# nmndeep/Robust-Segmentation

Measured on AMD Instinct MI355X. Metric: SEA attack-iterations/sec (UperNet-CNX-T, 512x512), higher is better.
Workload: dtype f32 (frozen-weight GEMMs on the 16-bit matrix cores by operand splitting: fp16x2 (22 significant bits per operand, 3 MFMA products) forward, fp16x2 (22 significant bits per operand, 3 MFMA products) input gradient; fp32 storage and accumulate)

## Files before the change

include/sea_hip.h:

```cpp
#ifndef SEA_HIP_H
#define SEA_HIP_H

#include <stddef.h>
#include <stdint.h>

#ifdef __cplusplus
extern "C" {
#endif

#define SEA_MODE_MASK_CE 0
#define SEA_MODE_MASK_CE_BAL 1
#define SEA_MODE_JS 2
#define SEA_MODE_CE 3

#define SEA_DTYPE_F32 0
#define SEA_DTYPE_BF16 1
#define SEA_DTYPE_F16 2

#define SEA_LAYOUT_NCHW 0
#define SEA_LAYOUT_NHWC 1

int sea_abi_version(void);
const char* sea_build_info(void);
#define SEA_CONFIG_XCD_ORDER 0
// ... 41 lines not shown
                     int64_t* tgt_cnt, void* stream);
int sea_confusion(const void* pred, int pred_bytes, const void* y, int y_bytes, int64_t n, int C,
                  int64_t* hist, void* stream);

int sea_apgd_track(const float* loss_sum, const float* track_sum, const int32_t* n_correct,
                   const int32_t* n_ignored, int B, int64_t HW, int iter, int n_iter, int check_k,
                   int early_stop, int init, int32_t* acc_cnt, float* acc, float* loss_best,
                   float* loss_best_last, float* reduced_last, float* step, float* loss_steps,
                   uint8_t* flags, int32_t* done, const void* loss_workspace, void* stream);
int sea_apgd_linf_step_graph(const float* x, float* x_adv, float* x_old, const float* grad, const float* step_b,
                             const float* eps_dev, const int32_t* iter_dev, int B, int64_t n_per_img, void* stream);
int sea_apgd_track_graph(const float* loss_sum, const float* track_sum, const int32_t* n_correct,
                         const int32_t* n_ignored, int B, int64_t HW, int32_t* iter_dev, const int32_t* check_table,
                         const int32_t* n_iter_dev, int early_stop, int32_t* acc_cnt, float* acc, float* loss_best,
                         float* loss_best_last, float* reduced_last, float* step, float* loss_steps, uint8_t* flags,
                         int32_t* done, const void* loss_workspace, void* stream);
int sea_select_copy(const uint8_t* flags, float* x_adv, float* grad, float* x_best,
                    float* grad_best, float* x_best_adv, const void* pred, void* pred_best,
                    int pred_bytes, int B, int64_t n_per_img, int64_t HW, void* stream);

int sea_count_ignored(const void* y, int y_bytes, int B, int64_t HW, int32_t* n_ignored,
                      void* stream);

int sea_worst_miou_greedy(const float* ints, const float* unions, int A, int N, int C,
                          uint32_t* mt_state, int n_rounds, double* miou, int32_t* selected,
                          int32_t* rounds_run);

int sea_dwconv7x7(const float* x, const float* w, const float* bias, float* y, int B, int C, int H,
                  int W, int flip, void* stream);
int sea_dwconv7x7_nhwc(const float* x, const float* wt, const float* bias, float* y, int B, int C,
                       int H, int W, int flip, unsigned ab, void* stream);
int sea_dwconv7x7_nhwc_add(const float* x, const float* wt, const float* bias, const float* addend, float* y, int B,
                           int C, int H, int W, int flip, unsigned ab, void* stream);

int sea_upsample_bilinear_fwd(const float* x, float* y, int64_t planes, int h, int w, int H, int W,
                              void* stream);
int sea_upsample_bilinear_bwd(const float* gy, float* gx, int64_t planes, int h, int w, int H, int W,
                              void* stream);
int sea_upsample_bilinear_nhwc_fwd(const float* x, const float* residual, float* y, int B, int C, int h,
                                   int w, int H, int W, int64_t y_pixel_stride, void* stream);
int sea_upsample_bilinear_nhwc_bwd(const float* gy, float* gx, int B, int C, int h, int w, int H, int W,
                                   int64_t gy_pixel_stride, void* stream);

int64_t sea_wino_tiles(int B, int H, int W, int m);
int sea_wino_input_transform(const float* x, int64_t x_pixel_stride, const float* gate, const float* scale,
                             float* V, int64_t v_tile_stride, int B, int C, int H, int W, int m, int vec4, void* stream);
int sea_wino_filter_transform(const float* w, float* U, int Cout, int Cin, int m, int flip, void* stream);
int sea_wino_input_transform_amax(const float* x, int64_t x_pixel_stride, const float* gate, const float* scale, float* V,
                                  int64_t v_tile_stride, int B, int C, int H, int W, int m, int vec4, uint32_t* amax_out,
                                  void* stream);
int sea_wino_output_transform(const float* M, const float* addend, const float* scale, const float* bias,
                              int relu, float* y, int B, int C, int H, int W, int m, int vec4, void* stream);

int sea_layernorm_fwd(const float* x, const float* w, const float* b, float* y, float* mean, float* rstd,
                      int64_t rows, int C, float eps, void* stream);
int sea_layernorm_bwd(const float* g, const float* x, const float* w, const float* mean, const float* rstd,
                      float* dx, int64_t rows, int C, void* stream);

int64_t sea_dwconv7x7_nhwc_wgrad_workspace(int B, int C, int H);
int sea_dwconv7x7_nhwc_wgrad(const float* x, const float* gy, float* gw, float* gb, float* ws, int B, int C, int H, int W,
                             void* stream);

int sea_adaptive_avg_pool_nhwc_fwd(const float* x, float* out, int B, int C, int H, int W, int oh, int ow, void* stream);
int sea_adaptive_avg_pool_nhwc_bwd(const float* g, float* dx, int B, int C, int H, int W, int oh, int ow, void* stream);

int sea_stem_conv1_ln_gelu(const float* x, const float* w, const float* bias, const float* gamma, const float* beta,
// ... 131 lines not shown
```

robust-segmentation_amd/csrc/dwconv_kernels.hip:

```cpp
#include "sea_common.h"

namespace sea {

constexpr int DW_T = 32;
constexpr int DW_K = 7, DW_P = 3;
constexpr int DW_IN = DW_T + DW_K - 1;
constexpr int DW_LD = 40;

template <bool FLIP, bool BIAS>
__global__ __launch_bounds__(256) void dwconv7x7_kernel(const float* __restrict__ x, const float* __restrict__ w,
                                                        const float* __restrict__ bias, float* __restrict__ y,
                                                        int C, int H, int W, int tiles_x) {
  __shared__ __attribute__((aligned(16))) float tile[DW_IN * DW_LD];
  const int plane = blockIdx.y;
  const int c = plane % C;
  const int ty0 = (blockIdx.x / tiles_x) * DW_T, tx0 = (blockIdx.x % tiles_x) * DW_T;
  const float* xp = x + (int64_t)plane * H * W;
  for (int i = threadIdx.x; i < DW_IN * DW_IN; i += 256) {
    const int r = i / DW_IN, q = i - r * DW_IN;
    const int gy = ty0 + r - DW_P, gx = tx0 + q - DW_P;
    float v = 0.f;
    if (gy >= 0 && gy < H && gx >= 0 && gx < W) v = xp[(int64_t)gy * W + gx];
    tile[r * DW_LD + q] = v;
  }
// ... 146 lines not shown
    float4 w[DW_K];
    load_input_row(oy0 - DW_P + r, in);
    if (r < DW_K) {
      load_filter_row(r, w);
      accumulate(in, w, acc0);
    }
    __builtin_amdgcn_sched_barrier(0);
    if (r >= 1) {
      load_filter_row(r - 1, w);
      accumulate(in, w, acc1);
    }
    __builtin_amdgcn_sched_barrier(0);
  }
  const int64_t ro = ((int64_t)b * H + oy0) * W * CG + cg;
  float4* yr = y + ro;
#pragma unroll
  for (int j = 0; j < DWN_STRIP; ++j)
    if (ox0 + j < W) {
      if (ADD) acc0[j] = add4(acc0[j], addend[ro + (int64_t)(ox0 + j) * CG]);
      yr[(int64_t)(ox0 + j) * CG] = acc0[j];
    }
  if (oy0 + 1 < H) {
#pragma unroll
    for (int j = 0; j < DWN_STRIP; ++j)
      if (ox0 + j < W) {
        if (ADD) acc1[j] = add4(acc1[j], addend[ro + ((int64_t)W + ox0 + j) * CG]);
        yr[((int64_t)W + ox0 + j) * CG] = acc1[j];
      }
  }
}

typedef float dw_f4 __attribute__((ext_vector_type(4)));

template <int CG, int ROWS, bool FLIP, bool BIAS, bool ADD, bool WLDS>
__global__ __launch_bounds__(256, 2) void dwconv7x7_nhwc_pipe_kernel(const float4* __restrict__ x, const float4* __restrict__ wt,
                                                                     const float4* __restrict__ bias,
                                                                     const float4* __restrict__ addend, float4* __restrict__ y,
                                                                     int H, int W, int gx, int HP, int units, int per_xcd) {
  constexpr int SPB = 256 / CG, NIN = DWN_STRIP + DW_K - 1;
  constexpr uint32_t OOB = 0x40000000u;
  extern __shared__ __attribute__((aligned(16))) char dw_smem[];
  const int cg = threadIdx.x % CG, ps = threadIdx.x / CG;
  const int u = per_xcd ? (int)(blockIdx.x % 8) * per_xcd + (int)(blockIdx.x / 8) : (int)blockIdx.x;
  if (u >= units) return;
  if constexpr (WLDS) {
    for (int i = threadIdx.x; i < DW_K * DW_K * CG; i += 256) {
      const int tap = i / CG, c = i - tap * CG;
      *(float4*)(dw_smem + i * 16) = wt[(FLIP ? (DW_K * DW_K - 1 - tap) : tap) * CG + c];
    }
    __syncthreads();
  }
  if (ps >= SPB) return;
  const int bx = u % gx, op = (u / gx) % HP, b = u / (gx * HP);
  const int oy0 = op * ROWS;
  const int ox0 = (bx * SPB + ps) * DWN_STRIP;
  if (ox0 >= W) return;
  const int row_bytes = W * CG * 16;
  const char* const img = (const char*)(x + (int64_t)b * H * W * CG);
  const uint32_t vbase = (uint32_t)((ox0 * CG + cg) * 16);
  const float4* const wb = wt + cg;

  dw_f4 in[2][NIN], w[2][DW_K];
  auto load_input_row = [&](int iy, dw_f4 (&dst)[NIN]) __attribute__((always_inline)) {
    const bool ok = iy >= 0 && iy < H;
    const __amdgpu_buffer_rsrc_t rs =
        __builtin_amdgcn_make_buffer_rsrc((void*)(img + (int64_t)(ok ? iy : 0) * row_bytes), 0, ok ? row_bytes : 0, 0x00020000);
#pragma unroll
    for (int j = 0; j < NIN; ++j) {
      uint32_t off;
      if (j < DW_P)
        off = ox0 > 0 ? vbase - (uint32_t)((DW_P - j) * CG * 16) : OOB;
      else
        off = vbase + (uint32_t)((j - DW_P) * CG * 16);
      dst[j] = __builtin_bit_cast(dw_f4, __builtin_amdgcn_raw_buffer_load_b128(rs, (int)off, 0, 0));
    }
  };
  auto load_filter_row = [&](int ky, dw_f4 (&dst)[DW_K]) __attribute__((always_inline)) {
#pragma unroll
    for (int kx = 0; kx < DW_K; ++kx) {
      const int tap = ky * DW_K + kx;
      if constexpr (WLDS)
        dst[kx] = *(const dw_f4*)(dw_smem + (tap * CG + cg) * 16);
      else
        dst[kx] = *(const dw_f4*)(wb + (FLIP ? (DW_K * DW_K - 1 - tap) : tap) * CG);
// ... 28 lines not shown
      if (r >= 1) accumulate(in[cur], w[cur ^ 1], acc1);
      __builtin_amdgcn_sched_barrier(0);
      if (r + 1 < DW_K) load_filter_row(r + 1, w[cur ^ 1]);
      __builtin_amdgcn_sched_barrier(0);
      if (r < DW_K) accumulate(in[cur], w[cur], acc0);
      __builtin_amdgcn_sched_barrier(0);
    }
  } else {
#pragma unroll
    for (int r = 0; r < DW_K; ++r) {
      const int cur = r & 1;
      if (r + 1 < DW_K) {
        load_input_row(oy0 - DW_P + r + 1, in[cur ^ 1]);
        load_filter_row(r + 1, w[cur ^ 1]);
      }
      __builtin_amdgcn_sched_barrier(0);
      accumulate(in[cur], w[cur], acc0);
      __builtin_amdgcn_sched_barrier(0);
    }
  }
  const int64_t ro = ((int64_t)b * H + oy0) * W * CG + cg;
  dw_f4* const yr = (dw_f4*)(y + ro);
#pragma unroll
  for (int j = 0; j < DWN_STRIP; ++j) {
    if (ADD) acc0[j] += *(const dw_f4*)(addend + ro + (int64_t)(ox0 + j) * CG);
    yr[(int64_t)(ox0 + j) * CG] = acc0[j];
  }
  if constexpr (ROWS == 2) {
#pragma unroll
    for (int j = 0; j < DWN_STRIP; ++j) {
      if (ADD) acc1[j] += *(const dw_f4*)(addend + ro + ((int64_t)W + ox0 + j) * CG);
      yr[((int64_t)W + ox0 + j) * CG] = acc1[j];
    }
  }
}

}

using namespace sea;

template <int CG, int ROWS, bool FLIP, bool BIAS, bool ADD>
static void dw_pipe_launch(dim3 grid, hipStream_t s, const float4* x4, const float4* w4, const float4* b4, const float4* a4,
                           float4* y4, int H, int W, int gx, int HP, int units, int per_xcd, bool wlds) {
  if constexpr (CG <= 96) {
    if (wlds) {
      constexpr int lds = DW_K * DW_K * CG * 16;
      auto k = dwconv7x7_nhwc_pipe_kernel<CG, ROWS, FLIP, BIAS, ADD, true>;
      if constexpr (lds > 65536) {
        static bool attr_set_dev[64] = {};
        int dev = 0;
        (void)hipGetDevice(&dev);
        if (!attr_set_dev[dev & 63]) {
          (void)hipFuncSetAttribute((const void*)k, hipFuncAttributeMaxDynamicSharedMemorySize, lds);
          attr_set_dev[dev & 63] = true;
        }
      }
      hipLaunchKernelGGL(k, grid, dim3(256), (size_t)lds, s, x4, w4, b4, a4, y4, H, W, gx, HP, units, per_xcd);
      return;
    }
  }
  hipLaunchKernelGGL((dwconv7x7_nhwc_pipe_kernel<CG, ROWS, FLIP, BIAS, ADD, false>), grid, dim3(256), 0, s, x4, w4, b4, a4, y4, H, W,
                     gx, HP, units, per_xcd);
}

extern "C" int sea_dwconv7x7_nhwc_add(const float* x, const float* wt, const float* bias, const float* addend, float* y,
                                      int B, int C, int H, int W, int flip, unsigned ab, void* stream) {
  SEA_CHECK_ARG(ab < 128 && !(ab & 1));
  SEA_CHECK_ARG(x && wt && y && B > 0 && B <= 65535 && C > 0 && (C % 4) == 0 && C <= 1024 && H > 0 && H <= 65535 && W > 0);
  SEA_CHECK_ARG(((((uintptr_t)x) | ((uintptr_t)wt) | ((uintptr_t)y) | ((uintptr_t)bias) | ((uintptr_t)addend)) & 15) == 0);
  SEA_CHECK_ARG(!(addend && bias));
  const int CG = C / 4;
  const int spb = 256 / CG;
  const int strips = (W + DWN_STRIP - 1) / DWN_STRIP;
  const int gx = (strips + spb - 1) / spb;
  hipStream_t s = (hipStream_t)stream;
  const float4 *x4 = (const float4*)x, *w4 = (const float4*)wt, *b4 = (const float4*)bias, *a4 = (const float4*)addend;
  float4* y4 = (float4*)y;
  const int CG0 = C / 4;
  const bool pipe_ok = !(ab & 16) && (CG0 == 24 || CG0 == 48 || CG0 == 96 || CG0 == 192) && (int64_t)B * H * W * C * 4 < (1ll << 31) &&
                       (W % DWN_STRIP) == 0;
  const bool two_rows = !(ab & 4) && H >= 2 && ((ab & 8) || (int64_t)H * W >= (pipe_ok && (H % 2) == 0 ? 1024 : 4096));
  const int HP = two_rows ? (H + 1) / 2 : H;
  const int64_t units64 = (int64_t)gx * HP * B;
  SEA_CHECK_ARG(units64 < (1ll << 30));
  const int units = (int)units64;
  const int per_xcd = (ab & 2) ? 0 : (units + 7) / 8;
  dim3 grid(per_xcd ? per_xcd * 8 : units), block(256);
#define SEA_DW_LAUNCH(F, BI, AD)                                                                                        \
  do {                                                                                                                  \
    if (two_rows)                                                                                                       \
      hipLaunchKernelGGL((dwconv7x7_nhwc_2row_kernel<F, BI, AD>), grid, block, 0, s, x4, w4, b4, a4, y4, CG, H, W, spb,  \
                         gx, HP, units, per_xcd);                                                                       \
    else                                                                                                                \
      hipLaunchKernelGGL((dwconv7x7_nhwc_kernel<F, BI, AD>), grid, block, 0, s, x4, w4, b4, a4, y4, CG, H, W, spb, gx,   \
                         units, per_xcd);                                                                               \
  } while (0)
  const bool piped = pipe_ok && (!two_rows || (H % 2) == 0);
#define SEA_DW_PIPE(CGV, F, BI, AD)                                                              \
  do {                                                                                           \
    if (two_rows)                                                                                \
      dw_pipe_launch<CGV, 2, F, BI, AD>(grid, s, x4, w4, b4, a4, y4, H, W, gx, HP, units, per_xcd, wlds); \
    else                                                                                         \
      dw_pipe_launch<CGV, 1, F, BI, AD>(grid, s, x4, w4, b4, a4, y4, H, W, gx, HP, units, per_xcd, wlds); \
  } while (0)
  const bool wlds = !(ab & 32) && (!two_rows || (ab & 64));
#define SEA_DW_PIPE_CG(F, BI, AD)                       \
  do {                                                  \
    if (CG == 24) SEA_DW_PIPE(24, F, BI, AD);           \
    else if (CG == 48) SEA_DW_PIPE(48, F, BI, AD);      \
    else if (CG == 96) SEA_DW_PIPE(96, F, BI, AD);      \
    else SEA_DW_PIPE(192, F, BI, AD);                   \
  } while (0)
  if (piped) {
    if (flip) {
      if (addend) SEA_DW_PIPE_CG(true, false, true); else SEA_DW_PIPE_CG(true, false, false);
    } else if (bias) {
      SEA_DW_PIPE_CG(false, true, false);
    } else if (addend) {
      SEA_DW_PIPE_CG(false, false, true);
    } else {
      SEA_DW_PIPE_CG(false, false, false);
    }
    SEA_RETURN_LAST();
  }
#undef SEA_DW_PIPE_CG
#undef SEA_DW_PIPE
  if (flip) {
    if (addend)
      SEA_DW_LAUNCH(true, false, true);
    else
      SEA_DW_LAUNCH(true, false, false);
  } else if (bias) {
    SEA_DW_LAUNCH(false, true, false);
  } else if (addend) {
    SEA_DW_LAUNCH(false, false, true);
  } else {
    SEA_DW_LAUNCH(false, false, false);
  }
#undef SEA_DW_LAUNCH
  SEA_RETURN_LAST();
}

namespace sea {
__global__ __launch_bounds__(448) void dwconv7x7_nhwc_wgrad_partial_kernel(const float4* __restrict__ x,
                                                                           const float4* __restrict__ gy,
// ... 91 lines not shown
  return R < 1 ? 1 : (R > 8 ? 8 : R);
}
static inline int dw_wgrad_chunks(int tiles) { return tiles >= 64 ? 32 : 1; }

extern "C" int64_t sea_dwconv7x7_nhwc_wgrad_workspace(int B, int C, int H) {
  if (B <= 0 || C <= 0 || H <= 0) return 0;
  const int R = dw_wgrad_rows(B, C, H);
  const int64_t tiles = (int64_t)B * ((H + R - 1) / R);
  return (tiles + 32) * 50 * C;
}

extern "C" int sea_dwconv7x7_nhwc_wgrad(const float* x, const float* gy, float* gw, float* gb, float* ws, int B, int C,
                                        int H, int W, void* stream) {
  SEA_CHECK_ARG(x && gy && gw && ws && B > 0 && C > 0 && (C % 4) == 0 && H > 0 && W > 0);
  SEA_CHECK_ARG(((((uintptr_t)x) | ((uintptr_t)gy) | ((uintptr_t)ws)) & 15) == 0);
  const int R = dw_wgrad_rows(B, C, H), tpi = (H + R - 1) / R;
  SEA_CHECK_ARG((int64_t)B * tpi < (1ll << 31));
  const int tiles = B * tpi, chunks = dw_wgrad_chunks(tiles), per = (tiles + chunks - 1) / chunks;
  hipStream_t st = (hipStream_t)stream;
  hipLaunchKernelGGL(dwconv7x7_nhwc_wgrad_partial_kernel, dim3(tiles, (C / 4 + 63) / 64), dim3(448), 0, st, (const float4*)x,
                     (const float4*)gy, (float4*)ws, C / 4, H, W, R, tpi);
  const dim3 g1((50 * C + 255) / 256, chunks), g2((50 * C + 255) / 256, 1);
  if (chunks > 1) {
    float* ws2 = ws + (int64_t)tiles * 50 * C;
    hipLaunchKernelGGL(dwconv7x7_nhwc_wgrad_reduce_kernel, g1, dim3(256), 0, st, (const float*)ws, ws2, (float*)nullptr,
                       (float*)nullptr, C, tiles, per);
    hipLaunchKernelGGL(dwconv7x7_nhwc_wgrad_reduce_kernel, g2, dim3(256), 0, st, (const float*)ws2, (float*)nullptr, gw, gb, C,
                       chunks, chunks);
  } else {
    hipLaunchKernelGGL(dwconv7x7_nhwc_wgrad_reduce_kernel, g2, dim3(256), 0, st, (const float*)ws, (float*)nullptr, gw, gb, C, tiles,
                       tiles);
  }
  SEA_RETURN_LAST();
}

extern "C" int sea_dwconv7x7_nhwc(const float* x, const float* wt, const float* bias, float* y, int B, int C, int H,
                                  int W, int flip, unsigned ab, void* stream) {
  return sea_dwconv7x7_nhwc_add(x, wt, bias, nullptr, y, B, C, H, W, flip, ab, stream);
}

extern "C" int sea_dwconv7x7(const float* x, const float* w, const float* bias, float* y, int B, int C, int H, int W,
                             int flip, void* stream) {
  SEA_CHECK_ARG(x && w && y && B > 0 && C > 0 && H > 0 && W > 0);
  const int64_t planes = (int64_t)B * C;
  SEA_CHECK_ARG(planes <= 65535 * 16);
  const int tiles_x = (W + DW_T - 1) / DW_T, tiles_y = (H + DW_T - 1) / DW_T;
  SEA_CHECK_ARG(planes <= 2147483647 / 1 && (int64_t)tiles_x * tiles_y <= 2147483647);
  hipStream_t s = (hipStream_t)stream;
  const int64_t chunk = 65535;
  for (int64_t p0 = 0; p0 < planes; p0 += chunk) {
    const int np = (int)((planes - p0) < chunk ? (planes - p0) : chunk);
    SEA_CHECK_ARG(p0 % C == 0 || planes <= chunk);
    dim3 grid(tiles_x * tiles_y, np);
    const float* xs = x + p0 * H * W;
    float* ys = y + p0 * H * W;
    if (flip)
      hipLaunchKernelGGL((dwconv7x7_kernel<true, false>), grid, dim3(256), 0, s, xs, w, (const float*)nullptr, ys, C, H, W, tiles_x);
    else if (bias)
      hipLaunchKernelGGL((dwconv7x7_kernel<false, true>), grid, dim3(256), 0, s, xs, w, bias, ys, C, H, W, tiles_x);
    else
      hipLaunchKernelGGL((dwconv7x7_kernel<false, false>), grid, dim3(256), 0, s, xs, w, (const float*)nullptr, ys, C, H, W, tiles_x);
  }
  SEA_RETURN_LAST();
}
```

robust-segmentation_amd/semseg/_native.py:

```python
from __future__ import annotations

import ctypes as C
import os
from typing import Optional

import torch

_PKG = os.path.dirname(os.path.dirname(os.path.abspath(__file__)))
LIB_PATH = os.environ.get("SEA_HIP_LIB", os.path.join(_PKG, "lib", "libsea_hip.so"))

MODE_BY_NAME = {"mask-ce-avg": 0, "mask-ce-bal": 1, "js-avg": 2, "ce": 3, "ce-avg": 3}
DTYPE_CODE = {torch.float32: 0, torch.bfloat16: 1, torch.float16: 2}
LAYOUT_NCHW, LAYOUT_NHWC = 0, 1

_lib = None

_vp, _i, _i64, _f, _sz, _u = C.c_void_p, C.c_int, C.c_int64, C.c_float, C.c_size_t, C.c_uint
_SIGS = {
    "sea_abi_version": (C.c_int, []),
    "sea_build_info": (C.c_char_p, []),
    "sea_fastdiv_magic": (_i, [C.c_uint32, C.POINTER(C.c_uint32), C.POINTER(C.c_uint32)]),
    "sea_apgd_linf_step": (_i, [_vp, _vp, _vp, _vp, _vp, _f, _f, _vp, _i, _i64, _vp]),
    "sea_apgd_l2_workspace_bytes": (_i64, [_i]),
    "sea_apgd_l2_step": (_i, [_vp, _vp, _vp, _vp, _vp, _f, _f, _vp, _vp, _i, _i64, _vp]),
    "sea_linf_random_start": (_i, [_vp, _vp, _f, _vp, _i64, _vp]),
    "sea_linf_project": (_i, [_vp, _vp, _f, _vp, _i64, _vp]),
    "sea_pgd_linf_step": (_i, [_vp, _vp, _vp, _f, _f, _vp, _vp, _i, _i64, _vp]),
    "sea_loss_workspace_bytes": (_sz, [_i, _i64]),
    "sea_loss_fwd_bwd": (_i, [_vp, _i, _i, _vp, _i, _vp, _i, _i, _i, _i, _i64, _f, _vp, _vp, _i, _vp, _vp, _sz,
                              _vp, _vp, _vp, _vp]),
    "sea_loss_fwd_bwd_tuned": (_i, [_vp, _i, _i, _vp, _i, _vp, _i, _i, _i, _i, _i64, _f, _vp, _vp, _i, _vp, _vp,
                                    _sz, _vp, _vp, _vp, _vp, _i]),
    "sea_loss_upsampled_workspace_bytes": (_sz, [_i, _i, _i, _i, _i, _i, _i]),
    "sea_loss_fwd_bwd_upsampled": (_i, [_vp, _vp, _i, _vp, _i, _i, _i, _i, _i, _i, _i, _i, _f, _vp, _vp, _i, _vp, _sz, _vp,
                                        _vp, _vp, _i, _vp]),
    "sea_class_counts": (_i, [_vp, _i, _vp, _i, _i, _i, _i64, _i, _i, _vp, _vp, _vp, _vp]),
    "sea_confusion": (_i, [_vp, _i, _vp, _i, _i64, _i, _vp, _vp]),
    "sea_apgd_track": (_i, [_vp, _vp, _vp, _vp, _i, _i64, _i, _i, _i, _i, _i, _vp, _vp, _vp, _vp, _vp, _vp, _vp,
                            _vp, _vp, _vp, _vp]),
    "sea_apgd_linf_step_graph": (_i, [_vp, _vp, _vp, _vp, _vp, _vp, _vp, _i, _i64, _vp]),
    "sea_apgd_track_graph": (_i, [_vp, _vp, _vp, _vp, _i, _i64, _vp, _vp, _vp, _i, _vp, _vp, _vp, _vp, _vp, _vp, _vp, _vp,
                                  _vp, _vp, _vp]),
    "sea_select_copy": (_i, [_vp, _vp, _vp, _vp, _vp, _vp, _vp, _vp, _i, _i, _i64, _i64, _vp]),
    "sea_count_ignored": (_i, [_vp, _i, _i, _i64, _vp, _vp]),
    "sea_worst_miou_greedy": (_i, [_vp, _vp, _i, _i, _i, _vp, _i, _vp, _vp, _vp]),
    "sea_dwconv7x7": (_i, [_vp, _vp, _vp, _vp, _i, _i, _i, _i, _i, _vp]),
    "sea_dwconv7x7_nhwc": (_i, [_vp, _vp, _vp, _vp, _i, _i, _i, _i, _i, _u, _vp]),
    "sea_dwconv7x7_nhwc_add": (_i, [_vp, _vp, _vp, _vp, _vp, _i, _i, _i, _i, _i, _u, _vp]),
    "sea_nchw_to_nhwc": (_i, [_vp, _vp, _vp, _i, _i, _i64, _vp]),
    "sea_nhwc_to_nchw": (_i, [_vp, _vp, _vp, _vp, _i, _i, _i64, _vp]),
    "sea_upsample_bilinear_fwd": (_i, [_vp, _vp, _i64, _i, _i, _i, _i, _vp]),
    "sea_upsample_bilinear_bwd": (_i, [_vp, _vp, _i64, _i, _i, _i, _i, _vp]),
    "sea_layernorm_fwd": (_i, [_vp, _vp, _vp, _vp, _vp, _vp, _i64, _i, _f, _vp]),
    "sea_layernorm_bwd": (_i, [_vp, _vp, _vp, _vp, _vp, _vp, _i64, _i, _vp]),
    "sea_dwconv7x7_nhwc_wgrad_workspace": (_i64, [_i, _i, _i]),
    "sea_dwconv7x7_nhwc_wgrad": (_i, [_vp, _vp, _vp, _vp, _vp, _i, _i, _i, _i, _vp]),
    "sea_adaptive_avg_pool_nhwc_fwd": (_i, [_vp, _vp, _i, _i, _i, _i, _i, _i, _vp]),
    "sea_adaptive_avg_pool_nhwc_bwd": (_i, [_vp, _vp, _i, _i, _i, _i, _i, _i, _vp]),
    "sea_stem_conv1_ln_gelu": (_i, [_vp, _vp, _vp, _vp, _vp, _vp, _vp, _i, _i, _i, _i, _f, _vp]),
    "sea_stem_conv1_bwd": (_i, [_vp, _vp, _vp, _i, _i, _i, _i, _vp]),
    "sea_ln_gelu_cl_fwd": (_i, [_vp, _vp, _vp, _vp, _i, _i, _i, _i64, _f, _vp]),
    "sea_ln_gelu_cl_bwd": (_i, [_vp, _i, _vp, _vp, _vp, _vp, _i, _i, _i64, _f, _vp]),
    "sea_wino_tiles": (_i64, [_i, _i, _i, _i]),
    "sea_wino_input_transform": (_i, [_vp, _i64, _vp, _vp, _vp, _i64, _i, _i, _i, _i, _i, _i, _vp]),
    "sea_wino_filter_transform": (_i, [_vp, _vp, _i, _i, _i, _i, _vp]),
    "sea_wino_output_transform": (_i, [_vp, _vp, _vp, _vp, _i, _vp, _i, _i, _i, _i, _i, _i, _vp]),
    "sea_tap_gather_fwd": (_i, [_vp, _vp, _i, _i, _i, _i, _i, _i, _i, _i, _vp]),
    "sea_tap_gather_bwd": (_i, [_vp, _vp, _i, _i, _i, _i, _i, _i, _vp]),
    "sea_gate_scale": (_i, [_vp, _vp, _vp, _vp, _i64, _i, _vp]),
    "sea_upsample_bilinear_nhwc_fwd": (_i, [_vp, _vp, _vp, _i, _i, _i, _i, _i, _i, _i64, _vp]),
    "sea_upsample_bilinear_nhwc_bwd": (_i, [_vp, _vp, _i, _i, _i, _i, _i, _i, _i64, _vp]),
    "sea_patch2x2": (_i, [_vp, _vp, _i, _i, _i, _i, _i, _vp]),
    "sea_attention_bwd_terms": (_i, [_vp, _vp, _vp, _i64, _i64, _i64, _i, _i, _i, _i, _f, _vp, _vp, _vp, _vp, _vp, _vp, _vp,
                                     _i64, _i64, _i64, _i, _vp]),
    "sea_attention_fwd_terms": (_i, [_vp, _vp, _vp, _i64, _i64, _i64, _i, _i, _i, _i, _f, _vp, _vp, _i, _vp]),
    "sea_attention_fwd_f16": (_i, [_vp, _vp, _vp, _i64, _i64, _i64, _i, _i, _i, _i, _f, _vp, _vp, _vp, _vp]),
    "sea_attention_bwd_f16": (_i, [_vp, _vp, _vp, _i64, _i64, _i64, _i, _i, _i, _i, _f, _vp, _vp, _vp, _vp, _vp, _vp, _vp, _vp,
                                   _i64, _i64, _i64, _vp]),
    "sea_absmax_bits": (_i, [_vp, _i64, _i, _i, _i, _i64, _i, _vp, _vp]),
    "sea_gemm_split_f16": (_i, [_vp, _i64, _vp, _vp, _i64, _vp, _i, _i, _i, _i, _i, _i64, _i64, _i64, _vp, _i, _vp, _u, _vp]),
    "sea_wino_input_transform_amax": (_i, [_vp, _i64, _vp, _vp, _vp, _i64, _i, _i, _i, _i, _i, _i, _vp, _vp]),
# ... 842 lines not shown
        if v_amax is not None:
            _check(L.sea_wino_input_transform_amax(_p(t), xps, _p(gate), _p(gate_scale), V.data_ptr() + 4 * off, Cin, B,
                                                   t.shape[1], H, W, m, WINO_IN_VEC4 & 1, _p(v_amax), _stream()),
                   "sea_wino_input_transform_amax")
        else:
            _check(L.sea_wino_input_transform(_p(t), xps, _p(gate), _p(gate_scale), V.data_ptr() + 4 * off, Cin, B, t.shape[1],
                                              H, W, m, WINO_IN_VEC4 & 1, _stream()), "sea_wino_input_transform")
        off += t.shape[1]
    if use_split:
        packed = U.__dict__.setdefault("_sea_packed", {})
        Up, ver = packed.get(gemm_terms, (None, None))
        if Up is None or ver != U._version:
            fresh = gemm_split_pack(U, trans=True, terms=gemm_terms)
            if Up is None or not Up.refresh_from(fresh):
                Up = fresh
                CACHE_EPOCH[0] += 1
            packed[gemm_terms] = (Up, U._version)
        Mx = gemm_split(V, Up, amax=v_amax, amax_rows=1 if v_amax is not None else 0, groups=B)
    else:
        with torch.autocast("cuda", enabled=False):
            Mx = _f32c(torch.bmm(V, U))
    del V
    y = torch.empty(B, Cout, H, W, dtype=torch.float32, device=xs[0].device, memory_format=torch.channels_last)
    if addend is not None and (tuple(addend.shape) != (B, Cout, H, W) or cl_pixel_stride(addend) != Cout):
        raise SeaNativeError("wino_conv3x3_cl: addend must be a dense channels_last (B,Cout,H,W) float32 tensor")
    _check(L.sea_wino_output_transform(_p(Mx), _p(addend), _p(scale), _p(bias), int(relu), _p(y), B, Cout, H, W, m,
                                       (WINO_IN_VEC4 >> 1) & 1, _stream()), "sea_wino_output_transform")
    return y


DWCONV_AB = int(os.environ.get("SEA_DWCONV_AB", "0"))


def dwconv7x7_nhwc(x, wt, bias=None, flip: bool = False, addend=None, ab: int = None):
    _dev(x, wt, bias, addend)
    B, H, W, Cc = x.shape
    if addend is not None and (addend.shape != x.shape or addend.dtype != torch.float32 or not addend.is_contiguous()):
        raise SeaNativeError("dwconv7x7_nhwc: addend must be a contiguous float32 tensor of the input's shape")
    y = torch.empty_like(x)
    _check(lib().sea_dwconv7x7_nhwc_add(_p(_f32c(x)), _p(_f32c(wt)), _p(bias), _p(addend), _p(y), B, Cc, H, W, int(flip),
                                        DWCONV_AB if ab is None else int(ab), _stream()), "sea_dwconv7x7_nhwc_add")
    return y


def dwconv7x7_nhwc_weight_grad(x, gy, want_bias: bool = True):
    _dev(x, gy)
    B, H, W, Cc = x.shape
    if gy.shape != x.shape or Cc % 4:
        raise SeaNativeError("dwconv7x7_nhwc_weight_grad: x and gy (B,H,W,C) of one shape, C % 4 == 0")
    L = lib()
    ws = torch.empty(int(L.sea_dwconv7x7_nhwc_wgrad_workspace(B, Cc, H)), dtype=torch.float32, device=x.device)
    gw = torch.empty((Cc, 1, 7, 7), dtype=torch.float32, device=x.device)
    gb = torch.empty(Cc, dtype=torch.float32, device=x.device) if want_bias else None
    _check(L.sea_dwconv7x7_nhwc_wgrad(_p(_f32c(x)), _p(_f32c(gy)), _p(gw), _p(gb), _p(ws), B, Cc, H, W, _stream()),
           "sea_dwconv7x7_nhwc_wgrad")
    return gw, gb


def nchw_to_nhwc(x, scale=None):
    _dev(x, scale)
    B, Cc, H, W = x.shape
    out = torch.empty(B, H, W, Cc, dtype=torch.float32, device=x.device)
    _check(lib().sea_nchw_to_nhwc(_p(_f32c(x)), _p(scale), _p(out), B, Cc, H * W, _stream()), "sea_nchw_to_nhwc")
    return out


def nhwc_to_nchw(y, scale=None, residual=None):
    _dev(y, scale, residual)
    B, H, W, Cc = y.shape
    out = torch.empty(B, Cc, H, W, dtype=torch.float32, device=y.device)
    _check(lib().sea_nhwc_to_nchw(_p(_f32c(y)), _p(scale), _p(None if residual is None else _f32c(residual)), _p(out),
                                  B, Cc, H * W, _stream()), "sea_nhwc_to_nchw")
# ... 288 lines not shown
KSPLIT_BELOW, KSPLIT_TARGET, KSPLIT_MIN_KB = (int(v) for v in os.environ.get("SEA_GEMM_KSPLIT_PARAMS", "400,768,8").split(","))
_ksplit_ws = {}


def _ksplit(M, N, K):
    blocks = -(-M // 128) * -(-N // 128)
    nkb = K // 32
    if not KSPLIT or blocks >= KSPLIT_BELOW or N % 4:
        return 1
    S = min(-(-KSPLIT_TARGET // blocks), nkb // KSPLIT_MIN_KB)
    while S > 1 and nkb % S:
        S -= 1
    return max(S, 1)


def _ksplit_workspace(device, numel):
    key = device.index if device.index is not None else torch.cuda.current_device()
    ws = _ksplit_ws.get(key)
    if ws is None or ws.numel() < numel:
        ws = _ksplit_ws[key] = torch.empty(numel, dtype=torch.float32, device=device)
    return ws[:numel]


def ksplit_workspace_pin(device):
    return _ksplit_ws.get(device.index if device.index is not None else torch.cuda.current_device())


class _GemmEpilogue(C.Structure):
    _fields_ = [("addend", C.c_void_p), ("ld_addend", C.c_int64), ("stride_addend", C.c_int64),
                ("gelu_out", C.c_void_p), ("gelu_grad_of", C.c_void_p), ("a_gelu_grad_of", C.c_void_p), ("a_gate", C.c_int), ("a_gelu", C.c_int),
                ("a_amax_mul", C.c_float), ("a_amax_mul_dev", C.c_void_p)]


def _amax_words(A3, M, K, G, sA, groups, per_row=False):
    if per_row and G != 1:
        raise SeaNativeError("gemm_split: row_amax (one scale word per row) is defined for a single matrix, not a batch of them")
    if per_row:
        words = torch.empty(M, dtype=torch.int32, device=A3.device)
        _check(lib().sea_absmax_bits(_p(A3), A3.stride(1), M, K, 1, 0, 1, _p(words), _stream()), "sea_absmax_bits")
        return words, 1
    rpw = M // groups if (groups > 1 and M % groups == 0) else 0
    words = torch.empty(groups if rpw else 1, dtype=torch.int32, device=A3.device)
    _check(lib().sea_absmax_bits(_p(A3), A3.stride(1), M, K, G, sA, rpw, _p(words), _stream()), "sea_absmax_bits")
    return words, rpw


_e = os.environ.get("SEA_GEMM_PIPE", "")
GEMM_PIPE = int(_e[0]) if _e[:1] in ("0", "1", "2", "3") else 2
GEMM_MFMA_SHAPE = 16 if os.environ.get("SEA_GEMM_SHAPE", "")[:1] == "1" else 32
del _e
_GEMM_PIPE_BITS = {2: 0, 0: 1, 1: 2, 3: 3}
_GEMM_SHAPE16 = 4


def gemm_variant(pipe=None, mfma_shape=None) -> int:
    pipe = GEMM_PIPE if pipe is None else int(pipe)
    mfma_shape = GEMM_MFMA_SHAPE if mfma_shape is None else int(mfma_shape)
    if pipe not in _GEMM_PIPE_BITS or mfma_shape not in (16, 32):
        raise SeaNativeError("gemm_split: pipe must be 0, 1, 2 or 3 and mfma_shape 16 or 32")
    return _GEMM_PIPE_BITS[pipe] | (_GEMM_SHAPE16 if mfma_shape == 16 else 0)


def gemm_split(A, Wp: PackedWeight, bias=None, relu: bool = False, out=None, amax=None, out_amax=None, addend=None,
               gelu_out=None, gelu_grad_of=None, amax_rows: int = 0, groups: int = 1, a_gelu_grad_of=None,
               a_gelu: bool = False, a_relu_gate=None, row_amax: bool = False, amax_mul: float = 1.0, pipe=None,
               mfma_shape=None):
    variant = gemm_variant(pipe, mfma_shape)
    gate = a_relu_gate is not None
    if gate:
        if a_gelu_grad_of is not None:
# ... 96 lines not shown
```

robust-segmentation_amd/semseg/models/convnext_upernet.py:

```python
from __future__ import annotations

import os

import torch
import torch.nn.functional as F
from torch import nn

CONVNEXT_SETTINGS = {
    "T": ([3, 3, 9, 3], [96, 192, 384, 768], 384, 0.4),
    "T_CVST": ([3, 3, 9, 3], [96, 192, 384, 768], 384, 0.4),
    "T_CVST_ROB": ([3, 3, 9, 3], [96, 192, 384, 768], 384, 0.4),
    "S_CVST": ([3, 3, 27, 3], [96, 192, 384, 768], 384, 0.3),
    "S_CVST_ROB": ([3, 3, 27, 3], [96, 192, 384, 768], 384, 0.3),
    "B": ([3, 3, 27, 3], [128, 256, 512, 1024], 512, 0.4),
}


def _fp32_fwd(fn):
    def forward(ctx, *args):
        if torch.is_autocast_enabled():
            args = [a.float() if (torch.is_tensor(a) and a.is_floating_point() and a.dtype != torch.float32) else a
                    for a in args]
            with torch.autocast("cuda", enabled=False):
                return fn(ctx, *args)
# ... 112 lines not shown

    @staticmethod
    @_fp32_fwd
    def forward(ctx, x, weight, bias, wt):
        from .. import _native as N
        ctx.save_for_backward(x, weight, wt)
        ctx.has_bias = bias is not None
        return N.dwconv7x7_nhwc(x, wt, bias, flip=False)

    @staticmethod
    @_fp32_bwd
    def backward(ctx, gy):
        from .. import _native as N
        x, weight, wt = ctx.saved_tensors
        gx = gw = gb = None
        gy = gy.contiguous()
        if ctx.needs_input_grad[0]:
            gx = N.dwconv7x7_nhwc(gy, wt, None, flip=True)
        if ctx.needs_input_grad[1]:
            gw, gb = _dw_weight_grad(x, weight, gy, ctx.has_bias and ctx.needs_input_grad[2])
        elif ctx.has_bias and ctx.needs_input_grad[2]:
            gb = gy.sum((0, 1, 2))
        return gx, gw, gb, None


class _DwConv7x7NHWCSkip(torch.autograd.Function):

    @staticmethod
    @_fp32_fwd
    def forward(ctx, x, weight, bias, wt):
        from .. import _native as N
        ctx.save_for_backward(x, weight, wt)
        ctx.has_bias = bias is not None
        return x.view_as(x), N.dwconv7x7_nhwc(x, wt, bias, flip=False)

    @staticmethod
    @_fp32_bwd
    def backward(ctx, g_skip, gy):
        from .. import _native as N
        x, weight, wt = ctx.saved_tensors
        gx = gw = gb = None
        if gy is None:
            return g_skip, None, None, None
        gy = gy.contiguous()
        if ctx.needs_input_grad[0]:
            add = None
            if g_skip is not None:
                add = g_skip if (g_skip.is_contiguous() and g_skip.dtype == torch.float32) else g_skip.float().contiguous()
            gx = N.dwconv7x7_nhwc(gy, wt, None, flip=True, addend=add)
        if ctx.needs_input_grad[1]:
            gw, gb = _dw_weight_grad(x, weight, gy, ctx.has_bias and ctx.needs_input_grad[2])
        elif ctx.has_bias and ctx.needs_input_grad[2]:
            gb = gy.sum((0, 1, 2))
        return gx, gw, gb, None


def _tkey(*ts):
    return tuple((id(t), t.data_ptr(), t._version, t.device.index) for t in ts if t is not None)


def _stable(old, new):
    from .. import _native as N
    if isinstance(new, N.PackedWeight):
        if isinstance(old, N.PackedWeight) and old.refresh_from(new):
            return old
        N.CACHE_EPOCH[0] += 1
        return new
    if isinstance(new, torch.Tensor):
        if (isinstance(old, torch.Tensor) and old is not new and old.shape == new.shape and old.dtype == new.dtype
                and old.device == new.device and old.stride() == new.stride()):
            old.copy_(new)
            return old
        N.CACHE_EPOCH[0] += 1
        return new
    if isinstance(new, (list, tuple)):
        olds = old if isinstance(old, (list, tuple)) and len(old) == len(new) else [None] * len(new)
        return type(new)(_stable(o, n) for o, n in zip(olds, new))
    return new


GEMM_TERMS = int(os.environ.get("SEA_GEMM_TERMS", "22"))
GEMM_TERMS_AUTOCAST = int(os.environ.get("SEA_GEMM_TERMS_AUTOCAST", "2"))
# ... 143 lines not shown
        r2 = None if res is None else res.reshape(-1, res.shape[-1])
        ctx.w, ctx.b1, ctx.caches, ctx.shape, ctx.terms, ctx.has_res = (w1, w2), b1, caches, x.shape, terms, res is not None
        ctx.fuse, ctx.a1 = fuse, a1
        rows_ok = lambda t: t.stride(1) == 1 and t.stride(0) % 4 == 0 and t.data_ptr() % 16 == 0
        if (terms == 22 and fuse & 16 and a1 is not None and a2 is not None and a1.numel() == 1 and a2.numel() == 1
                and b1 is not None and N.mlp_fused_ok(w2.shape[0], w1.shape[0]) and rows_ok(x2)
                and (r2 is None or rows_ok(r2))):
            y = N.mlp_fused_forward(x2, _packed(w1, caches[0], "lin_fwd", False, terms), b1,
                                    _packed(w2, caches[1], "lin_fwd", False, terms), b2, r2, a1, a2, ln=ln)
            ctx.kernel_fused, ctx.ln = True, ln
            ctx.save_for_backward(x2)
            return y.view(x.shape)
        if ln is not None:
            raise RuntimeError("_FrozenMlp: a LayerNorm was handed in but the fused kernel does not apply (see _mlp_takes_layernorm)")
        ctx.kernel_fused = False
        t = torch.empty(x2.shape[0], w1.shape[0], dtype=torch.float32, device=x.device)
        pro = bool(fuse & 16) and -(-w2.shape[0] // 128) <= FUSE_PROLOGUE_MAX_NBLOCKS and not fuse & 1
        if pro:
            N.gemm_split(x2, _packed(w1, caches[0], "lin_fwd", False, terms), bias=b1, out=t, amax=a1, groups=nb)
            h = t
        elif fuse & 1:
            h = torch.empty_like(t)
            N.gemm_split(x2, _packed(w1, caches[0], "lin_fwd", False, terms), bias=b1, out=t, gelu_out=h, amax=a1, groups=nb)
        else:
            N.gemm_split(x2, _packed(w1, caches[0], "lin_fwd", False, terms), bias=b1, out=t, amax=a1, groups=nb)
            h = F.gelu(t)
        split2 = REDUCE_ADD and N._ksplit(x2.shape[0], w2.shape[0], w2.shape[1]) > 1
        add_in = r2 is not None and r2.is_contiguous() and (split2 or (bool(fuse & 4) and not pro))
        y = N.gemm_split(t if pro else h, _packed(w2, caches[1], "lin_fwd", False, terms), bias=b2, amax=a2, groups=nb,
                         a_gelu=pro, addend=r2 if add_in else None)
        if r2 is not None and not add_in:
            y += r2
        ctx.save_for_backward(t)
        return y.view(x.shape)

    @staticmethod
    @_fp32_bwd
    def backward(ctx, g):
        from .. import _native as N
        (t,) = ctx.saved_tensors
        terms = _bwd_terms(ctx.terms)
        g2 = g.reshape(-1, g.shape[-1])
        if not g2.is_contiguous():
            g2 = g2.contiguous()
        nb = ctx.shape[0] if len(ctx.shape) > 2 else 1
        if ctx.kernel_fused:
            x2 = t
            p1f = _packed(ctx.w[0], ctx.caches[0], "lin_fwd", False, ctx.terms)
            if terms == 22 and g2.data_ptr() % 16 == 0:
                gx = N.mlp_fused_backward(g2, x2, p1f, ctx.b1, _packed(ctx.w[1], ctx.caches[1], "lin_bwd", True, terms),
                                          _packed(ctx.w[0], ctx.caches[0], "lin_bwd", True, terms), ctx.a1,
                                          _l1_bound(ctx.w[1], ctx.caches[1], dim=0, factor=1.13), ln=ctx.ln)
                return gx.view(ctx.shape), None, None, None, None, (g if ctx.has_res else None), None, None, None, None
            if ctx.ln is not None:
                xin = x2
                x2, ln_mean, ln_rstd = N.layernorm(xin, ctx.ln[0], ctx.ln[1], ctx.ln[2])
            t = N.gemm_split(x2, p1f, bias=ctx.b1, amax=ctx.a1, groups=nb)
        p2, p1 = (_packed(ctx.w[1], ctx.caches[1], "lin_bwd", True, terms), _packed(ctx.w[0], ctx.caches[0], "lin_bwd", True, terms))
        rows = {}
        if terms == 22:
            words, _ = N._amax_words(g2.unsqueeze(0), g2.shape[0], g2.shape[1], 1, 0, nb, per_row=True)
            rows = dict(amax=words, amax_rows=1)
            mul = dict(amax_mul=_l1_bound(ctx.w[1], ctx.caches[1], dim=0, factor=1.13), **rows)
        else:
            mul = {}
        if ctx.fuse & 2:
# ... 212 lines not shown
                y = self.act(_linear_frozen(gc[0], self.norm(y), self.pwconv1.weight, self.pwconv1.bias, amax=a1))
                y = self.pwconv2(y)
                if g is not None:
                    y = g * y
            return (xn + y).permute(0, 3, 1, 2)
        y = depthwise7x7(self.dwconv, x)
        if no_drop and _fast_layout_ok(x) and y.is_contiguous():
            y = self.pwconv2(self.act(self.pwconv1(self.norm(_ToNHWC.apply(y)))))
            return _ScaleResidual.apply(x, y, self.gamma)
        y = y.permute(0, 2, 3, 1)
        y = self.pwconv2(self.act(self.pwconv1(self.norm(y))))
        if self.gamma is not None:
            y = self.gamma * y
        return x + self.drop_path(y.permute(0, 3, 1, 2))


class _PatchConv2x2(torch.autograd.Function):

    @staticmethod
    def forward(ctx, x, weight, bias, cache, amax=None):
        B, C, H, W = x.shape
        key = _tkey(weight)
        if cache.get("key") != key:
            cache.update(key=key, w=_stable(cache.get("w"), weight.detach().permute(0, 2, 3, 1).reshape(weight.shape[0], 4 * C).contiguous()))
        wr = cache["w"]
        from .. import _native as N
        xn = x.permute(0, 2, 3, 1)
        if xn.is_contiguous() and xn.dtype == torch.float32 and C % 4 == 0:
            patches = N.patch2x2(xn)
        else:
            patches = xn.reshape(B, H // 2, 2, W // 2, 2, C).permute(0, 1, 3, 2, 4, 5).reshape(-1, 4 * C)
        y = _frozen_mm(patches, wr, cache, "patch_fwd", bias=bias, amax=amax, groups=B)
        ctx.wr, ctx.shape, ctx.cache, ctx.terms = wr, (B, C, H, W), cache, _terms()
        return y.float().view(B, H // 2, W // 2, -1).permute(0, 3, 1, 2)

    @staticmethod
    def backward(ctx, gy):
        B, C, H, W = ctx.shape
        g = gy.permute(0, 2, 3, 1).reshape(-1, gy.shape[1])
        rows = _frozen_mm(g if g.is_contiguous() else g.contiguous(), ctx.wr, ctx.cache, "patch_bwd", trans=True,
                          terms=_bwd_terms(ctx.terms), groups=B, row_amax=True).float()
        if C % 4 == 0 and rows.is_contiguous():
            from .. import _native as N
            gp = N.unpatch2x2(rows, B, H, W)
        else:
            gp = rows.view(B, H // 2, W // 2, 2, 2, C).permute(0, 1, 3, 2, 4, 5).reshape(B, H, W, C)
        return gp.permute(0, 3, 1, 2), None, None, None, None


def _patch_conv_ok(conv, x):
    return (USE_HIP_DWCONV and isinstance(conv, nn.Conv2d) and conv.kernel_size == (2, 2) and conv.stride == (2, 2)
            and conv.padding == (0, 0) and conv.groups == 1 and x.is_cuda and x.dtype == torch.float32
            and conv.weight.dtype == torch.float32
            and x.shape[2] % 2 == 0 and x.shape[3] % 2 == 0
            and not (conv.weight.requires_grad or (conv.bias is not None and conv.bias.requires_grad)))


class ConvNeXt(nn.Module):
    def __init__(self, strr: str, in_chans: int = 3, layer_scale_init_value: float = 1.0, out_indices=(0, 1, 2, 3)):
        super().__init__()
        if strr not in CONVNEXT_SETTINGS:
            raise AssertionError(f"ConvNeXt model name should be in {list(CONVNEXT_SETTINGS)}")
        depths, dims, _, dpr = CONVNEXT_SETTINGS[strr]
        self.variant = strr
        self.downsample_layers = nn.ModuleList()
        if "CVST" in strr:
# ... 633 lines not shown
```

Before: 552.2.

## Fuse per-row absmax scale computation into backward depthwise conv epilogue

The backward 7x7 depthwise conv (flipped, with skip addend) now also computes the per-pixel absolute-max bit word of its output in its epilogue, using lane shuffles and LDS atomics. The word is published through a module-level slot so the next split-precision GEMM's row_amax path can take it instead of launching a separate absmax pass over the gradient. This removes one extra kernel and a full re-read of the activation gradient per block. In exchange the dwconv epilogue gains reductions and atomics, and a fragile pointer/version handshake between autograd forward and backward is introduced.

```diff
diff --git a/include/sea_hip.h b/include/sea_hip.h
--- a/include/sea_hip.h
+++ b/include/sea_hip.h
@@ -97,6 +97,8 @@
                        int H, int W, int flip, unsigned ab, void* stream);
 int sea_dwconv7x7_nhwc_add(const float* x, const float* wt, const float* bias, const float* addend, float* y, int B,
                            int C, int H, int W, int flip, unsigned ab, void* stream);
+int sea_dwconv7x7_nhwc_rows(const float* x, const float* wt, const float* bias, const float* addend, float* y,
+                            uint32_t* row_amax, int B, int C, int H, int W, int flip, unsigned ab, void* stream);
 
 int sea_upsample_bilinear_fwd(const float* x, float* y, int64_t planes, int h, int w, int H, int W,
                               void* stream);
diff --git a/robust-segmentation_amd/csrc/dwconv_kernels.hip b/robust-segmentation_amd/csrc/dwconv_kernels.hip
--- a/robust-segmentation_amd/csrc/dwconv_kernels.hip
+++ b/robust-segmentation_amd/csrc/dwconv_kernels.hip
@@ -202,24 +202,14 @@
 
 typedef float dw_f4 __attribute__((ext_vector_type(4)));
 
-template <int CG, int ROWS, bool FLIP, bool BIAS, bool ADD, bool WLDS>
-__global__ __launch_bounds__(256, 2) void dwconv7x7_nhwc_pipe_kernel(const float4* __restrict__ x, const float4* __restrict__ wt,
-                                                                     const float4* __restrict__ bias,
-                                                                     const float4* __restrict__ addend, float4* __restrict__ y,
-                                                                     int H, int W, int gx, int HP, int units, int per_xcd) {
+template <int CG, int ROWS, bool FLIP, bool BIAS, bool ADD, bool WLDS, bool ROWMAX>
+__device__ __forceinline__ void dw_pipe_tile(const float4* __restrict__ x, const float4* __restrict__ wt,
+                                             const float4* __restrict__ bias, const float4* __restrict__ addend,
+                                             float4* __restrict__ y, int H, int W, int gx, int HP, int u, const char* dw_smem,
+                                             uint32_t* pmax) {
   constexpr int SPB = 256 / CG, NIN = DWN_STRIP + DW_K - 1;
   constexpr uint32_t OOB = 0x40000000u;
-  extern __shared__ __attribute__((aligned(16))) char dw_smem[];
   const int cg = threadIdx.x % CG, ps = threadIdx.x / CG;
-  const int u = per_xcd ? (int)(blockIdx.x % 8) * per_xcd + (int)(blockIdx.x / 8) : (int)blockIdx.x;
-  if (u >= units) return;
-  if constexpr (WLDS) {
-    for (int i = threadIdx.x; i < DW_K * DW_K * CG; i += 256) {
-      const int tap = i / CG, c = i - tap * CG;
-      *(float4*)(dw_smem + i * 16) = wt[(FLIP ? (DW_K * DW_K - 1 - tap) : tap) * CG + c];
-    }
-    __syncthreads();
-  }
   if (ps >= SPB) return;
   const int bx = u % gx, op = (u / gx) % HP, b = u / (gx * HP);
   const int oy0 = op * ROWS;
@@ -314,6 +304,81 @@
       if (ADD) acc1[j] += *(const dw_f4*)(addend + ro + ((int64_t)W + ox0 + j) * CG);
       yr[((int64_t)W + ox0 + j) * CG] = acc1[j];
     }
+  }
+  if constexpr (ROWMAX) {
+    static_assert(CG % 8 == 0 && DWN_STRIP == 8, "a pixel's lanes come in whole groups of eight");
+    auto bits4 = [](const dw_f4 v) __attribute__((always_inline)) {
+      uint32_t m = 0;
+#pragma unroll
+      for (int e = 0; e < 4; ++e) {
+        const uint32_t b = __float_as_uint(v[e]) & 0x7fffffffu;
+        m = b > m ? b : m;
+      }
+#pragma unroll
+      for (int o = 1; o < 8; o <<= 1) {
+        const uint32_t other = (uint32_t)__shfl_xor((int)m, o, 64);
+        m = other > m ? other : m;
+      }
+      return m;
+    };
+    const bool first = (threadIdx.x & 7) == 0;
+#pragma unroll
+    for (int j = 0; j < DWN_STRIP; ++j) {
+      const uint32_t m0 = bits4(acc0[j]);
+      if (first) atomicMax(pmax + (ps * ROWS) * DWN_STRIP + j, m0);
+      if constexpr (ROWS == 2) {
+        const uint32_t m1 = bits4(acc1[j]);
+        if (first) atomicMax(pmax + (ps * ROWS + 1) * DWN_STRIP + j, m1);
+      }
+    }
+  }
+}
+
+template <int CG, int ROWS, bool FLIP, bool BIAS, bool ADD, bool WLDS>
+__global__ __launch_bounds__(256, 2) void dwconv7x7_nhwc_pipe_kernel(const float4* __restrict__ x, const float4* __restrict__ wt,
+                                                                     const float4* __restrict__ bias,
+                                                                     const float4* __restrict__ addend, float4* __restrict__ y,
+                                                                     int H, int W, int gx, int HP, int units, int per_xcd) {
+  extern __shared__ __attribute__((aligned(16))) char dw_smem[];
+  const int u = per_xcd ? (int)(blockIdx.x % 8) * per_xcd + (int)(blockIdx.x / 8) : (int)blockIdx.x;
+  if (u >= units) return;
+  if constexpr (WLDS) {
+    for (int i = threadIdx.x; i < DW_K * DW_K * CG; i += 256) {
+      const int tap = i / CG, c = i - tap * CG;
+      *(float4*)(dw_smem + i * 16) = wt[(FLIP ? (DW_K * DW_K - 1 - tap) : tap) * CG + c];
+    }
+    __syncthreads();
+  }
+  dw_pipe_tile<CG, ROWS, FLIP, BIAS, ADD, WLDS, false>(x, wt, bias, addend, y, H, W, gx, HP, u, dw_smem, nullptr);
+}
+
+template <int CG, int ROWS, bool WLDS>
+__global__ __launch_bounds__(256, 2) void dwconv7x7_nhwc_pipe_rows_kernel(const float4* __restrict__ x,
+                                                                          const float4* __restrict__ wt,
+                                                                          const float4* __restrict__ addend,
+                                                                          float4* __restrict__ y, uint32_t* __restrict__ row_amax,
+                                                                          int H, int W, int gx, int HP, int units, int per_xcd) {
+  constexpr int SPB = 256 / CG, NPIX = SPB * ROWS * DWN_STRIP;
+  static_assert(NPIX <= 256, "one lane per pixel word");
+  extern __shared__ __attribute__((aligned(16))) char dw_smem[];
+  __shared__ uint32_t pmax[NPIX];
+  const int u = per_xcd ? (int)(blockIdx.x % 8) * per_xcd + (int)(blockIdx.x / 8) : (int)blockIdx.x;
+  if (u >= units) return;
+  if (threadIdx.x < NPIX) pmax[threadIdx.x] = 0u;
+  if constexpr (WLDS) {
+    for (int i = threadIdx.x; i < DW_K * DW_K * CG; i += 256) {
+      const int tap = i / CG, c = i - tap * CG;
+      *(float4*)(dw_smem + i * 16) = wt[(DW_K * DW_K - 1 - tap) * CG + c];
+    }
+  }
+  __syncthreads();
+  dw_pipe_tile<CG, ROWS, true, false, true, WLDS, true>(x, wt, nullptr, addend, y, H, W, gx, HP, u, dw_smem, pmax);
+  __syncthreads();
+  if (threadIdx.x < NPIX) {
+    const int bx = u % gx, op = (u / gx) % HP, b = u / (gx * HP);
+    const int ps = threadIdx.x / (ROWS * DWN_STRIP), r = (threadIdx.x / DWN_STRIP) % ROWS, j = threadIdx.x % DWN_STRIP;
+    const int oy = op * ROWS + r, ox = (bx * SPB + ps) * DWN_STRIP + j;
+    if (oy < H && ox < W) row_amax[((int64_t)b * H + oy) * W + ox] = pmax[threadIdx.x];
   }
 }
 
@@ -345,8 +410,32 @@
                      gx, HP, units, per_xcd);
 }
 
-extern "C" int sea_dwconv7x7_nhwc_add(const float* x, const float* wt, const float* bias, const float* addend, float* y,
-                                      int B, int C, int H, int W, int flip, unsigned ab, void* stream) {
+template <int CG, int ROWS>
+static void dw_pipe_rows_launch(dim3 grid, hipStream_t s, const float4* x4, const float4* w4, const float4* a4, float4* y4,
+                                uint32_t* row_amax, int H, int W, int gx, int HP, int units, int per_xcd, bool wlds) {
+  if constexpr (CG <= 96) {
+    if (wlds) {
+      constexpr int lds = DW_K * DW_K * CG * 16;
+      auto k = dwconv7x7_nhwc_pipe_rows_kernel<CG, ROWS, true>;
+      if constexpr (lds > 65536 - 1024) {
+        static bool attr_set_dev[64] = {};
+        int dev = 0;
+        (void)hipGetDevice(&dev);
+        if (!attr_set_dev[dev & 63]) {
+          (void)hipFuncSetAttribute((const void*)k, hipFuncAttributeMaxDynamicSharedMemorySize, lds);
+          attr_set_dev[dev & 63] = true;
+        }
+      }
+      hipLaunchKernelGGL(k, grid, dim3(256), (size_t)lds, s, x4, w4, a4, y4, row_amax, H, W, gx, HP, units, per_xcd);
+      return;
+    }
+  }
+  hipLaunchKernelGGL((dwconv7x7_nhwc_pipe_rows_kernel<CG, ROWS, false>), grid, dim3(256), 0, s, x4, w4, a4, y4, row_amax, H, W, gx,
+                     HP, units, per_xcd);
+}
+
+static int dwconv7x7_nhwc_impl(const float* x, const float* wt, const float* bias, const float* addend, float* y,
+                               uint32_t* row_amax, int B, int C, int H, int W, int flip, unsigned ab, void* stream) {
   SEA_CHECK_ARG(ab < 128 && !(ab & 1));
   SEA_CHECK_ARG(x && wt && y && B > 0 && B <= 65535 && C > 0 && (C % 4) == 0 && C <= 1024 && H > 0 && H <= 65535 && W > 0);
   SEA_CHECK_ARG(((((uintptr_t)x) | ((uintptr_t)wt) | ((uintptr_t)y) | ((uintptr_t)bias) | ((uintptr_t)addend)) & 15) == 0);
@@ -393,6 +482,27 @@
     else if (CG == 96) SEA_DW_PIPE(96, F, BI, AD);      \
     else SEA_DW_PIPE(192, F, BI, AD);                   \
   } while (0)
+  if (piped && row_amax != nullptr && flip && addend) {
+#define SEA_DW_ROWS(CGV)                                                                                              \
+  do {                                                                                                                \
+    if (two_rows)                                                                                                     \
+      dw_pipe_rows_launch<CGV, 2>(grid, s, x4, w4, a4, y4, row_amax, H, W, gx, HP, units, per_xcd, wlds);              \
+    else                                                                                                              \
+      dw_pipe_rows_launch<CGV, 1>(grid, s, x4, w4, a4, y4, row_amax, H, W, gx, HP, units, per_xcd, wlds);              \
+  } while (0)
+    if (CG == 24) SEA_DW_ROWS(24);
+    else if (CG == 48) SEA_DW_ROWS(48);
+    else if (CG == 96) SEA_DW_ROWS(96);
+    else SEA_DW_ROWS(192);
+#undef SEA_DW_ROWS
+    SEA_RETURN_LAST();
+  }
+  if (row_amax != nullptr) {
+    SEA_CHECK_ARG((int64_t)B * H * W < (1ll << 31));
+    const int rc = dwconv7x7_nhwc_impl(x, wt, bias, addend, y, nullptr, B, C, H, W, flip, ab, stream);
+    if (rc != 0) return rc;
+    return sea_absmax_bits(y, C, B * H * W, C, 1, 0, 1, row_amax, stream);
+  }
   if (piped) {
     if (flip) {
       if (addend) SEA_DW_PIPE_CG(true, false, true); else SEA_DW_PIPE_CG(true, false, false);
@@ -550,6 +660,17 @@
                        tiles);
   }
   SEA_RETURN_LAST();
+}
+
+extern "C" int sea_dwconv7x7_nhwc_add(const float* x, const float* wt, const float* bias, const float* addend, float* y,
+                                      int B, int C, int H, int W, int flip, unsigned ab, void* stream) {
+  return dwconv7x7_nhwc_impl(x, wt, bias, addend, y, nullptr, B, C, H, W, flip, ab, stream);
+}
+
+extern "C" int sea_dwconv7x7_nhwc_rows(const float* x, const float* wt, const float* bias, const float* addend, float* y,
+                                       uint32_t* row_amax, int B, int C, int H, int W, int flip, unsigned ab, void* stream) {
+  SEA_CHECK_ARG(row_amax != nullptr);
+  return dwconv7x7_nhwc_impl(x, wt, bias, addend, y, row_amax, B, C, H, W, flip, ab, stream);
 }
 
 extern "C" int sea_dwconv7x7_nhwc(const float* x, const float* wt, const float* bias, float* y, int B, int C, int H,
diff --git a/robust-segmentation_amd/semseg/_native.py b/robust-segmentation_amd/semseg/_native.py
--- a/robust-segmentation_amd/semseg/_native.py
+++ b/robust-segmentation_amd/semseg/_native.py
@@ -47,6 +47,7 @@
     "sea_dwconv7x7": (_i, [_vp, _vp, _vp, _vp, _i, _i, _i, _i, _i, _vp]),
     "sea_dwconv7x7_nhwc": (_i, [_vp, _vp, _vp, _vp, _i, _i, _i, _i, _i, _u, _vp]),
     "sea_dwconv7x7_nhwc_add": (_i, [_vp, _vp, _vp, _vp, _vp, _i, _i, _i, _i, _i, _u, _vp]),
+    "sea_dwconv7x7_nhwc_rows": (_i, [_vp, _vp, _vp, _vp, _vp, _vp, _i, _i, _i, _i, _i, _u, _vp]),
     "sea_nchw_to_nhwc": (_i, [_vp, _vp, _vp, _i, _i, _i64, _vp]),
     "sea_nhwc_to_nchw": (_i, [_vp, _vp, _vp, _vp, _i, _i, _i64, _vp]),
     "sea_upsample_bilinear_fwd": (_i, [_vp, _vp, _i64, _i, _i, _i, _i, _vp]),
@@ -955,12 +956,18 @@
 DWCONV_AB = int(os.environ.get("SEA_DWCONV_AB", "0"))
 
 
-def dwconv7x7_nhwc(x, wt, bias=None, flip: bool = False, addend=None, ab: int = None):
+def dwconv7x7_nhwc(x, wt, bias=None, flip: bool = False, addend=None, ab: int = None, row_amax: bool = False):
     _dev(x, wt, bias, addend)
     B, H, W, Cc = x.shape
     if addend is not None and (addend.shape != x.shape or addend.dtype != torch.float32 or not addend.is_contiguous()):
         raise SeaNativeError("dwconv7x7_nhwc: addend must be a contiguous float32 tensor of the input's shape")
     y = torch.empty_like(x)
+    if row_amax:
+        words = torch.empty(B * H * W, dtype=torch.int32, device=x.device)
+        _check(lib().sea_dwconv7x7_nhwc_rows(_p(_f32c(x)), _p(_f32c(wt)), _p(bias), _p(addend), _p(y), _p(words), B, Cc, H, W,
+                                             int(flip), DWCONV_AB if ab is None else int(ab), _stream()),
+               "sea_dwconv7x7_nhwc_rows")
+        return y, words
     _check(lib().sea_dwconv7x7_nhwc_add(_p(_f32c(x)), _p(_f32c(wt)), _p(bias), _p(addend), _p(y), B, Cc, H, W, int(flip),
                                         DWCONV_AB if ab is None else int(ab), _stream()), "sea_dwconv7x7_nhwc_add")
     return y
@@ -1315,10 +1322,49 @@
                 ("a_amax_mul", C.c_float), ("a_amax_mul_dev", C.c_void_p)]
 
 
+ROW_WORDS_FROM_PRODUCERS = True
+ROW_WORDS_TAKEN = [0]
+_row_words_want = [None]
+_row_words_slot = [None]
+
+
+def row_words_want(y):
+    _row_words_want[0] = y.data_ptr() if (ROW_WORDS_FROM_PRODUCERS and y is not None and y.is_cuda) else None
+
+
+def row_words_wanted(x) -> bool:
+    want, _row_words_want[0] = _row_words_want[0], None
+    return want is not None and want == x.data_ptr()
+
+
+def row_words_publish(t, words):
+    _row_words_slot[0] = (t, t._version, words)
+
+
+def row_words_reset():
+    _row_words_want[0] = _row_words_slot[0] = None
+
+
+def _row_words_take(A2, M, K):
+    entry, _row_words_slot[0] = _row_words_slot[0], None
+    if entry is None:
+        return None
+    t, version, words = entry
+    if (t.data_ptr() == A2.data_ptr() and t.untyped_storage().data_ptr() == A2.untyped_storage().data_ptr()
+            and t._version == version and t.is_contiguous() and t.dtype == A2.dtype == torch.float32 and t.shape[-1] == K
+            and t.numel() == M * K and tuple(A2.shape) == (M, K) and A2.stride() == (K, 1) and words.numel() == M):
+        ROW_WORDS_TAKEN[0] += 1
+        return words
+    return None
+
+
 def _amax_words(A3, M, K, G, sA, groups, per_row=False):
     if per_row and G != 1:
         raise SeaNativeError("gemm_split: row_amax (one scale word per row) is defined for a single matrix, not a batch of them")
     if per_row:
+        words = _row_words_take(A3[0], M, K)
+        if words is not None:
+            return words, 1
         words = torch.empty(M, dtype=torch.int32, device=A3.device)
         _check(lib().sea_absmax_bits(_p(A3), A3.stride(1), M, K, 1, 0, 1, _p(words), _stream()), "sea_absmax_bits")
         return words, 1
diff --git a/robust-segmentation_amd/semseg/models/convnext_upernet.py b/robust-segmentation_amd/semseg/models/convnext_upernet.py
--- a/robust-segmentation_amd/semseg/models/convnext_upernet.py
+++ b/robust-segmentation_amd/semseg/models/convnext_upernet.py
@@ -168,6 +168,7 @@
         from .. import _native as N
         ctx.save_for_backward(x, weight, wt)
         ctx.has_bias = bias is not None
+        ctx.row_words = N.row_words_wanted(x)
         return x.view_as(x), N.dwconv7x7_nhwc(x, wt, bias, flip=False)
 
     @staticmethod
@@ -183,7 +184,11 @@
             add = None
             if g_skip is not None:
                 add = g_skip if (g_skip.is_contiguous() and g_skip.dtype == torch.float32) else g_skip.float().contiguous()
-            gx = N.dwconv7x7_nhwc(gy, wt, None, flip=True, addend=add)
+            if ctx.row_words and add is not None:
+                gx, words = N.dwconv7x7_nhwc(gy, wt, None, flip=True, addend=add, row_amax=True)
+                N.row_words_publish(gx, words)
+            else:
+                gx = N.dwconv7x7_nhwc(gy, wt, None, flip=True, addend=add)
         if ctx.needs_input_grad[1]:
             gw, gb = _dw_weight_grad(x, weight, gy, ctx.has_bias and ctx.needs_input_grad[2])
         elif ctx.has_bias and ctx.needs_input_grad[2]:
@@ -393,6 +398,8 @@
         if r2 is not None and not add_in:
             y += r2
         ctx.save_for_backward(t)
+        if _bwd_terms(terms) == 22:
+            N.row_words_want(y)
         return y.view(x.shape)
 
     @staticmethod
@@ -671,6 +678,8 @@
             patches = xn.reshape(B, H // 2, 2, W // 2, 2, C).permute(0, 1, 3, 2, 4, 5).reshape(-1, 4 * C)
         y = _frozen_mm(patches, wr, cache, "patch_fwd", bias=bias, amax=amax, groups=B)
         ctx.wr, ctx.shape, ctx.cache, ctx.terms = wr, (B, C, H, W), cache, _terms()
+        if _bwd_terms(ctx.terms) == 22 and y.dtype == torch.float32 and _split_ok(y, y.shape[1], 22):
+            N.row_words_want(y)
         return y.float().view(B, H // 2, W // 2, -1).permute(0, 3, 1, 2)
 
     @staticmethod
```

Result: no change. 552.0 (-0.0%).
